# gargatik/Seamless-Through-Breaking-Rethinking-Image-Stitching-for-Optimal-Alignment

Hardware: AMD Instinct MI355X
Metric: stitched image-pairs/s at 512x512 (higher is better)
Workload: dtype f32 (decoder contractions, PatchEmbed's third conv and the C = 128 block tails: exact 3xbf16 split of both operands, 6 products on the bf16 matrix cores, fp32 accumulate -- error vs fp64 0.83x the fp32 MFMA chain's; everything else fp32); 1 GPU; UDIS-D-shaped 512x512 pairs, batch=1, FlowHomoAdpater.forward(type=test_eval); launch=hipGraph replay, pairs_in_flight=3

## Files before the change

include/stitch_gfx950.h:

```cpp
#ifndef STITCH_GFX950_H
#define STITCH_GFX950_H
#include <stdint.h>
#ifdef __cplusplus
extern "C" {
#endif

typedef struct st_gemm_desc {
    const float* a;
    const float* w;
    float* c;
    const float* bias;
    const float* aux0;
    const float* aux1;
    const float* aux2;
    const float* scale_ptr;
    int32_t M, N, K;
    int32_t H, W, Cin, ldx;
    int32_t kh, kw, sh, sw, ph, pw, Ho, Wo;
    int32_t ldw, ldc, ld_aux0, ld_aux1, ld_aux2;
    int32_t aux0_row_div, aux0_row_mod;
    int32_t act;
    int32_t epi;
    float alpha;
    int32_t batch;
// ... 92 lines not shown
int st_corr_volume_both_plan(int32_t B, int32_t N, int32_t C, int32_t aligned16);

int st_layernorm(const float* x, int32_t ldx, const float* w, const float* b, float* out, int32_t ldo,
                 int32_t rows, int32_t C, float eps, void* stream);
int st_softmax_rows(float* x, int32_t ld, int32_t rows, int32_t C, void* stream);
int st_l2norm_rows(const float* x, float* out, int32_t rows, int32_t C, void* stream);
int st_maxpool_nhwc(const float* x, float* out, int32_t B, int32_t H, int32_t W, int32_t C, int32_t k,
                    int32_t s, int32_t p, void* stream);
int st_dwconv3x3_residual(const float* x, const float* w, const float* bias, float* out, int32_t B,
                          int32_t H, int32_t W, int32_t C, void* stream);
int st_sine_pe(float* out, int32_t ld, int32_t rows, int32_t dim, const float* coords, int32_t ldc,
               int32_t Wg, int32_t ws, int32_t period, float cscale, float coff, int32_t accumulate,
               void* stream);
int st_attention_small(const float* q, int64_t q_bs, int64_t q_ts, const float* k, int64_t k_bs, int64_t k_ts,
                       const float* v, int64_t v_bs, int64_t v_ts, float* out, int64_t o_bs, int64_t o_ts,
                       int32_t B, int32_t heads, int32_t Nq, int32_t Nk, int32_t D, float scale, void* stream);
int st_attention_kvlds(const float* q, int64_t q_bs, int64_t q_ts, const float* k, int64_t k_bs, int64_t k_ts,
                       const float* v, int64_t v_bs, int64_t v_ts, float* out, int64_t o_bs, int64_t o_ts,
                       int32_t B, int32_t heads, int32_t Nq, int32_t Nk, int32_t D, float scale, void* stream);
int st_window_attention(const float* q, const float* k, const float* v, int64_t bs, int64_t ts,
                        const float* qpad, const float* kpad, const float* vpad, float* out, int64_t o_bs,
                        int64_t o_ts, int32_t B, int32_t H, int32_t W, int32_t heads, int32_t D, int32_t ws,
                        float scale, void* stream);
int st_ccl_softargmax(const float* G, float* out, int32_t ldo, int32_t B, int32_t h, int32_t w, void* stream);
int st_patch_conv1(const float* maps, const float* w36x16, const float* bias, float* out, int32_t M, int32_t H,
                   int32_t W, int32_t Ho, int32_t Wo, void* stream);
int st_patch_conv12(const float* cost_maps, const float* c0_w36x16, const float* c0_b, const float* c2_w32x576,
                    const float* c2_b, float* s2, int32_t M, int32_t H, int32_t W, void* stream);
int st_patch_conv12_planes(const float* cost_maps, const float* c0_w36x16, const float* c0_b, const float* c2_w32x576, const float* c2_b,
                           void* s2_planes, int64_t s2_pstride, int32_t M, int32_t H, int32_t W, void* stream);
int st_copy2d(const float* src, int32_t lds, float* dst, int32_t ldd, int32_t rows, int32_t cols, void* stream);
int st_prep_image(const float* src, float* dst, int32_t B, int32_t C, int32_t H, int32_t W, int32_t ldo,
                  float mul, float div, float sub, void* stream);

int st_latent_pool(const float* scores, int32_t ld_s, const float* tokens, int32_t ld_t, float* z, int32_t pixels,
                   int32_t P, void* stream);

int st_coords_grid(float* out, int32_t B, int32_t H, int32_t W, void* stream);
int st_coords_grid_init(float* out, const float* init, int32_t B, int32_t H, int32_t W, void* stream);
int st_flow_forward_interpolate(const float* src, int32_t src_is_coords_rows, float* out, int32_t B, int32_t H, int32_t W,
                                void* stream);
int st_flow_from_coords(const float* coords1, float* flow4, int32_t ld4, float* dst2, int32_t ld2, int32_t B,
                        int32_t H, int32_t W, void* stream);
int st_flow_encode(const float* coords1, const float* w98, const float* bias, float* out, int32_t ldo, float* flow2,
                   int32_t ld2, int32_t B, int32_t H, int32_t W, int32_t Co, void* stream);
int st_flow_encode_split3(const float* coords1, const float* w98, const float* bias, float* out, int32_t ldo, float* flow2,
                          int32_t ld2, int32_t B, int32_t H, int32_t W, int32_t Co, void* out_planes, int64_t out_pstride,
                          int64_t out_prows, void* flow_planes, int64_t flow_pstride, int64_t flow_prows, int32_t flow_col,
                          void* stream);
int st_cost_lookup(const float* maps, const float* coords, float* out, int32_t ldo, int32_t Nq, int32_t H2,
                   int32_t W2, int32_t r, void* stream);
int st_decoder_token_chain(float* corr, int32_t ld_corr, const float* coords1, const float* kv,
                           const float* const* weights16, int32_t rows, int32_t ntok, void* stream);
int st_convex_upsample(const float* coords1, const float* mask, int32_t ldm, float* out, int32_t B, int32_t H,
                       int32_t W, void* stream);

int st_dlt4(const float* src4x2, const float* motion, float* H, int32_t B, float mscale_x, float mscale_y,
            float div, void* stream);
int st_mat3_sandwich(const float* L, const float* X, const float* R, float* out, int32_t B, int32_t invert,
                     void* stream);
int st_homo_warp(const float* U, const float* theta, float* out, int32_t* idx, int32_t B, int32_t C,
                 int32_t n_ones, int32_t H, int32_t W, int32_t oh, int32_t ow, void* stream);
int st_mesh_bounds(const float* H, float* out4, int32_t B, float width, float height, int32_t gw, int32_t gh,
                   void* stream);
int st_flow_warp(const float* x, const float* flow, const float* mul, float* out, int32_t B, int32_t C,
                 int32_t H, int32_t W, void* stream);
int st_homo_flow_warp(const float* image2, const float* H8, const float* flow, float* out6, float* overlap, float* Hi,
                      int32_t B, int32_t H, int32_t W, void* stream);
int st_resize_bilinear(const float* x, float* out, int32_t planes, int32_t H, int32_t W, int32_t oh, int32_t ow,
                       int32_t align_corners, float div0, float div1, int32_t ndiv, void* stream);
int st_range_map(const float* flow, void* scratch_u64, float* out, int32_t B, int32_t H, int32_t W, void* stream);
int st_occlusion_from_range(const float* range, float* out, int64_t n, int32_t threshold, void* stream);
int st_morph_open(const float* mask, float* out, void* scratch_u8x2, int32_t N, int32_t H, int32_t W,
                  int32_t ksz, void* stream);
int st_eval_finish(float* final6, const float* occ, float* overlap, int32_t B, int32_t H, int32_t W, void* stream);
int st_blend(const float* homo1, const float* homo2, float* fin, const float* occ, float* output2, float* mask1,
             float* mask2, uint8_t* blend, int32_t h, int32_t w, void* stream);
int st_blend_plain(const float* homo1, const float* homo2, const float* fin, float* output2, float* mask1, float* mask2,
                   uint8_t* blend, int32_t h, int32_t w, void* stream);
int st_mean_threshold(const float* x, float* out, int32_t B, int32_t C, int32_t H, int32_t W, float thr,
                      void* stream);
int st_tps_solve_grid(const float* U, const float* source, const float* target, void* work_f64, float* T,
                      float* out, int32_t* idx, int32_t B, int32_t C, int32_t H, int32_t W, int32_t N,
                      int32_t oh, int32_t ow, void* stream);

int st_masked_psnr_ssim(const float* image1, const float* warped, int64_t warped_batch_stride, const float* maskmean,
                        void* partial_f64, double* out_psnr_ssim, int32_t B, int32_t H, int32_t W, void* stream);
int st_channel_mean(const float* x, int64_t batch_stride, float* out, int32_t B, int32_t C, int32_t H, int32_t W,
                    void* stream);

int st_load_rgb8(const void* src_u8_hwc, float* dst_chw, int32_t B, int32_t H, int32_t W, void* stream);

int st_jpeg_workspace_bytes(int32_t H, int32_t W, int32_t channels);
int st_jpeg_max_bytes(int32_t H, int32_t W, int32_t channels);
int st_jpeg_encode_u8(const void* src, int32_t H, int32_t W, int32_t channels, int64_t row_stride, void* out, int64_t out_capacity,
                      int32_t* out_nbytes, void* workspace, int64_t workspace_bytes, void* stream);

typedef struct st_jpeg_enc_params {
    int32_t quality;
    int32_t hs, vs;
    int32_t optimize;
    int32_t reserved[4];
} st_jpeg_enc_params;
int st_abi_jpeg_enc_params_size(void);
int st_jpeg_workspace_bytes_ex(int32_t H, int32_t W, int32_t channels, const st_jpeg_enc_params* params);
int st_jpeg_max_bytes_ex(int32_t H, int32_t W, int32_t channels, const st_jpeg_enc_params* params);
// ... 123 lines not shown
```

seamless-through-breaking-rethinking-image-stitching-for-optimal-alignment_amd/csrc/flowops.hip:

```cpp
#include "common.h"
#include <type_traits>
#include "../../include/stitch_gfx950.h"

__global__ void coords_grid_kernel(float* __restrict__ out, int B, int H, int W) {
    const size_t idx = (size_t)blockIdx.x * blockDim.x + threadIdx.x;
    if (idx >= (size_t)B * H * W) return;
    const int r = idx % ((size_t)H * W);
    out[idx * 2] = (float)(r % W);
    out[idx * 2 + 1] = (float)(r / W);
}

extern "C" int st_coords_grid(float* out, int32_t B, int32_t H, int32_t W, void* stream) {
    if (!out || B <= 0 || H <= 0 || W <= 0) return ST_EINVAL;
    const size_t total = (size_t)B * H * W;
    hipLaunchKernelGGL(coords_grid_kernel, dim3((total + 255) / 256), dim3(256), 0, (hipStream_t)stream, out, B, H, W);
    ST_CHECK_LAUNCH();
    return ST_OK;
}

__global__ void coords_grid_init_kernel(float* __restrict__ out, const float* __restrict__ init, int B, int H, int W) {
    const size_t idx = (size_t)blockIdx.x * blockDim.x + threadIdx.x;
    if (idx >= (size_t)B * H * W) return;
    const size_t N = (size_t)H * W, b = idx / N;
    const int r = idx % N;
// ... 109 lines not shown
                const unsigned nh = (unsigned)__builtin_amdgcn_update_dpp(0, (int)ph, 0xB1, 0xF, 0xF, false);
                const unsigned nm = (unsigned)__builtin_amdgcn_update_dpp(0, (int)pm, 0xB1, 0xF, 0xF, false);
                const unsigned nl = (unsigned)__builtin_amdgcn_update_dpp(0, (int)pl, 0xB1, 0xF, 0xF, false);
                if (!(c & 1)) {
                    unsigned* pp = reinterpret_cast<unsigned*>(out_planes + ((size_t)(c >> 5) * out_prows + img + (size_t)y * W + x) * 32 + (c & 31));
                    pp[0] = ph | (nh << 16); pp[out_pstride / 2] = pm | (nm << 16); pp[out_pstride] = pl | (nl << 16);
                }
            }
        }
    }
    if (flow2 && blockIdx.y == 0 && (wave & 1) == 0 && lane < 8 && tx * 8 + lane < W) {
        const float2 f = patch[(row + 3) * 14 + lane + 3];
        const size_t r = img + (size_t)y * W + tx * 8 + lane;
        flow2[r * ld2] = f.x; flow2[r * ld2 + 1] = f.y;
        if (flow_planes) {
            __bf16 hx, mx, lx, hy, my, ly;
            unsigned* pp = reinterpret_cast<unsigned*>(flow_planes + ((size_t)(flow_col >> 5) * flow_prows + r) * 32 + (flow_col & 31));
            st_split3(f.x, hx, mx, lx);
            st_split3(f.y, hy, my, ly);
            pp[0] = st_bf16_bits(hx) | ((unsigned)st_bf16_bits(hy) << 16);
            pp[flow_pstride / 2] = st_bf16_bits(mx) | ((unsigned)st_bf16_bits(my) << 16);
            pp[flow_pstride] = st_bf16_bits(lx) | ((unsigned)st_bf16_bits(ly) << 16);
        }
    }
}

extern "C" int st_flow_encode(const float* coords1, const float* w98, const float* bias, float* out, int32_t ldo, float* flow2,
                              int32_t ld2, int32_t B, int32_t H, int32_t W, int32_t Co, void* stream) {
    if (!coords1 || !w98 || !bias || !out || B <= 0 || H <= 0 || W <= 0 || Co <= 0 || (Co & 3) || ((uintptr_t)w98 & 15)) return ST_EINVAL;
    if (ldo < Co || (flow2 && ld2 < 2) || ((uintptr_t)coords1 & 7)) return ST_EINVAL;
    dim3 grid(((H + 3) / 4) * ((W + 7) / 8), (Co + 127) / 128, B);
    hipLaunchKernelGGL(flow_encode_kernel, grid, dim3(512), 0, (hipStream_t)stream, coords1, w98, bias, out, ldo, flow2, ld2, H, W, Co,
                       (__bf16*)nullptr, 0LL, 0LL, (__bf16*)nullptr, 0LL, 0LL, 0);
    ST_CHECK_LAUNCH();
    return ST_OK;
}

extern "C" int st_flow_encode_split3(const float* coords1, const float* w98, const float* bias, float* out, int32_t ldo, float* flow2,
                                     int32_t ld2, int32_t B, int32_t H, int32_t W, int32_t Co, void* out_planes, int64_t out_pstride,
                                     int64_t out_prows, void* flow_planes, int64_t flow_pstride, int64_t flow_prows, int32_t flow_col,
                                     void* stream) {
    if (!coords1 || !w98 || !bias || !out || B <= 0 || H <= 0 || W <= 0 || Co <= 0 || (Co & 31) || ((uintptr_t)w98 & 15)) return ST_EINVAL;
    if (ldo < Co || (flow2 && ld2 < 2) || ((uintptr_t)coords1 & 7)) return ST_EINVAL;
    if (!out_planes || out_pstride <= 0 || out_prows < (int64_t)B * H * W) return ST_EINVAL;
    if (flow_planes && (!flow2 || flow_pstride <= 0 || flow_prows < (int64_t)B * H * W || flow_col < 0 || (flow_col & 1))) return ST_EINVAL;
    dim3 grid(((H + 3) / 4) * ((W + 7) / 8), (Co + 127) / 128, B);
    hipLaunchKernelGGL(flow_encode_kernel, grid, dim3(512), 0, (hipStream_t)stream, coords1, w98, bias, out, ldo, flow2, ld2, H, W, Co,
                       (__bf16*)out_planes, (long long)out_pstride, (long long)out_prows, (__bf16*)flow_planes, (long long)flow_pstride,
                       (long long)flow_prows, (int)flow_col);
    ST_CHECK_LAUNCH();
    return ST_OK;
}

__global__ __launch_bounds__(256) void cost_lookup_kernel(const float* __restrict__ maps, const float* __restrict__ coords,
                                                          float* __restrict__ out, int ldo, int Nq, int H2, int W2, int r) {
#pragma clang fp contract(off)
    const int side = 2 * r + 1, nch = side * side;
    const size_t idx = (size_t)blockIdx.x * 256 + threadIdx.x;
    if (idx >= (size_t)Nq * nch) return;
    const int ch = idx % nch;
    const size_t n = idx / nch;
    const int i = ch / side, j = ch % side;
    const float x = coords[n * 2] + (float)(i - r);
    const float y = coords[n * 2 + 1] + (float)(j - r);
    const float gx = 2.0f * x / (float)(W2 - 1) - 1.0f, gy = 2.0f * y / (float)(H2 - 1) - 1.0f;
    const float ix = ((gx + 1.0f) / 2.0f) * (float)(W2 - 1), iy = ((gy + 1.0f) / 2.0f) * (float)(H2 - 1);
    const float x0f = floorf(ix), y0f = floorf(iy);
    const int x0 = (int)x0f, y0 = (int)y0f, x1 = x0 + 1, y1 = y0 + 1;
    const float x1f = x0f + 1.0f, y1f = y0f + 1.0f;
    const float nw = (x1f - ix) * (y1f - iy), ne = (ix - x0f) * (y1f - iy);
    const float sw = (x1f - ix) * (iy - y0f), se = (ix - x0f) * (iy - y0f);
    const float* m = maps + n * (size_t)(H2 * W2);
    const bool xin0 = x0 >= 0 && x0 < W2, xin1 = x1 >= 0 && x1 < W2;
    const bool yin0 = y0 >= 0 && y0 < H2, yin1 = y1 >= 0 && y1 < H2;
    float v = (xin0 && yin0 ? m[y0 * W2 + x0] : 0.f) * nw;
    v = __fmaf_rn(xin1 && yin0 ? m[y0 * W2 + x1] : 0.f, ne, v);
    v = __fmaf_rn(xin0 && yin1 ? m[y1 * W2 + x0] : 0.f, sw, v);
    v = __fmaf_rn(xin1 && yin1 ? m[y1 * W2 + x1] : 0.f, se, v);
    out[n * ldo + ch] = v;
}

extern "C" int st_cost_lookup(const float* maps, const float* coords, float* out, int32_t ldo, int32_t Nq, int32_t H2,
                              int32_t W2, int32_t r, void* stream) {
    if (!maps || !coords || !out || Nq <= 0 || r < 0 || r > 64 || ldo < (2 * r + 1) * (2 * r + 1)) return ST_EINVAL;
    if (H2 < 2 || W2 < 2 || (int64_t)H2 * W2 > 0x7fffffff) return ST_EINVAL;
    const size_t total = (size_t)Nq * (2 * r + 1) * (2 * r + 1);
    hipLaunchKernelGGL(cost_lookup_kernel, dim3((total + 255) / 256), dim3(256), 0, (hipStream_t)stream, maps, coords, out,
                       ldo, Nq, H2, W2, r);
    ST_CHECK_LAUNCH();
    return ST_OK;
}

__global__ __launch_bounds__(256) void convex_upsample_kernel(const float* __restrict__ coords1, const float* __restrict__ mask,
                                                              int ldm, float* __restrict__ out, int B, int H, int W) {
    const size_t gid = (size_t)blockIdx.x * 256 + threadIdx.x;
    const size_t pix = gid >> 6;
    if (pix >= (size_t)B * H * W) return;
    const int sub = gid & 63, i = sub >> 3, j = sub & 7;
    const int b = pix / ((size_t)H * W), r = pix % ((size_t)H * W);
    const int y = r / W, x = r % W;
    const float* mp = mask + pix * ldm + sub;
    float mv[9], mx = -INFINITY;
#pragma unroll
    for (int k = 0; k < 9; ++k) { mv[k] = mp[k * 64]; mx = fmaxf(mx, mv[k]); }
    float sum = 0.f;
#pragma unroll
    for (int k = 0; k < 9; ++k) { mv[k] = expf(mv[k] - mx); sum += mv[k]; }
    float ox = 0.f, oy = 0.f;
#pragma unroll
    for (int k = 0; k < 9; ++k) {
        const int yy = y + k / 3 - 1, xx = x + k % 3 - 1;
        const bool ok = yy >= 0 && yy < H && xx >= 0 && xx < W;
        const size_t p2 = ((size_t)b * H + min(max(yy, 0), H - 1)) * W + min(max(xx, 0), W - 1);
        const float2 cxy = *reinterpret_cast<const float2*>(coords1 + p2 * 2);
        const float okf = ok ? 8.0f : 0.0f;
        const float fx = okf * (cxy.x - (float)xx), fy = okf * (cxy.y - (float)yy);
        const float wgt = mv[k] / sum;
        ox += wgt * fx; oy += wgt * fy;
    }
    const size_t HW8 = (size_t)64 * H * W;
    const size_t o = (size_t)b * 2 * HW8 + (size_t)(8 * y + i) * (8 * W) + (8 * x + j);
    out[o] = ox;
    out[o + HW8] = oy;
}

extern "C" int st_convex_upsample(const float* coords1, const float* mask, int32_t ldm, float* out, int32_t B, int32_t H,
                                  int32_t W, void* stream) {
    if (!coords1 || !mask || !out || ldm < 576 || B <= 0 || H <= 0 || W <= 0 || ((uintptr_t)coords1 & 7)) return ST_EINVAL;
    const size_t total = (size_t)B * H * W * 64;
    hipLaunchKernelGGL(convex_upsample_kernel, dim3((total + 255) / 256), dim3(256), 0, (hipStream_t)stream, coords1, mask,
                       ldm, out, B, H, W);
    ST_CHECK_LAUNCH();
// ... 22 lines not shown
#pragma unroll
    for (int j = 0; j < K / 16; ++j) {
        const float4 a = *reinterpret_cast<const float4*>(X + i * LDX + 16 * j + 4 * g);
        float4 b[2];
#pragma unroll
        for (int t = 0; t < 2; ++t) b[t] = *reinterpret_cast<const float4*>(Wh + (16 * t + i) * LDWT + 16 * j + 4 * g);
#pragma unroll
        for (int t = 0; t < 2; ++t) acc[t] = __builtin_amdgcn_mfma_f32_16x16x4f32(a.x, b[t].x, acc[t], 0, 0, 0);
#pragma unroll
        for (int t = 0; t < 2; ++t) acc[t] = __builtin_amdgcn_mfma_f32_16x16x4f32(a.y, b[t].y, acc[t], 0, 0, 0);
#pragma unroll
        for (int t = 0; t < 2; ++t) acc[t] = __builtin_amdgcn_mfma_f32_16x16x4f32(a.z, b[t].z, acc[t], 0, 0, 0);
#pragma unroll
        for (int t = 0; t < 2; ++t) acc[t] = __builtin_amdgcn_mfma_f32_16x16x4f32(a.w, b[t].w, acc[t], 0, 0, 0);
    }
}

__device__ __forceinline__ void tc_store2(float* __restrict__ X, const f32x4 v[2], int col0, int lane) {
    const int c = lane & 15, g = lane >> 4;
#pragma unroll
    for (int t = 0; t < 2; ++t)
#pragma unroll
        for (int r = 0; r < 4; ++r) X[(4 * g + r) * TC_LDW + col0 + 16 * t + c] = v[t][r];
}

__device__ __forceinline__ void tc_layernorm2(f32x4 v[2], const float* __restrict__ w, const float* __restrict__ b, float* __restrict__ red_mine,
                                              const float* __restrict__ red_other, int col0, int lane) {
    const int c = lane & 15, g = lane >> 4;
    float mh[4], m2h[4];
#pragma unroll
    for (int r = 0; r < 4; ++r) {
        mh[r] = sum16(v[0][r] + v[1][r]) * (1.0f / 32.0f);
        const float d0 = v[0][r] - mh[r], d1 = v[1][r] - mh[r];
        m2h[r] = sum16(d0 * d0 + d1 * d1);
        if (c == 0) { red_mine[(4 * g + r) * 2] = mh[r]; red_mine[(4 * g + r) * 2 + 1] = m2h[r]; }
    }
    __syncthreads();
#pragma unroll
    for (int r = 0; r < 4; ++r) {
        const float mo = red_other[(4 * g + r) * 2], m2o = red_other[(4 * g + r) * 2 + 1];
        const float mean = 0.5f * (mh[r] + mo), d = mh[r] - mo;
        const float var = ((m2h[r] + m2o) + d * d * 16.0f) * (1.0f / 64.0f);
        const float rstd = 1.0f / sqrtf(var + 1e-5f);
#pragma unroll
        for (int t = 0; t < 2; ++t) v[t][r] = (v[t][r] - mean) * rstd * w[col0 + 16 * t + c] + b[col0 + 16 * t + c];
    }
}

template <int I, int N, class F>
__device__ __forceinline__ void tc_static_for(F&& f) {
    if constexpr (I < N) { f(std::integral_constant<int, I>{}); tc_static_for<I + 1, N>(f); }
}

template <int RG>
__global__ __launch_bounds__(128 * RG) void decoder_token_chain_kernel(float* __restrict__ corr, int ldc, const float* __restrict__ coords1,
                                                                       const float* __restrict__ kv, TokenChainArgs A, int rows, int ntok) {
    extern __shared__ __attribute__((aligned(16))) float sm[];
    float* W0 = sm;
    float* W2 = W0 + 64 * TC_LDW0;
    float* Wq = W2 + 64 * TC_LDW;
    float* Wp = Wq + 64 * TC_LDW;
    float* Wf0 = Wp + 64 * TC_LDW;
    float* Wf3 = Wf0 + 64 * TC_LDW;
    float* Vec = Wf3 + 64 * TC_LDW;
    float* Slab = Vec + 10 * 64;
    float* Red = Slab + RG * 16 * (TC_LDW0 + TC_LDW);
    const int tid = threadIdx.x, lane = tid & 63, wave = tid >> 6;
    constexpr int NT = 128 * RG;
    const int rg = wave >> 1, hf = wave & 1, col0 = 32 * hf;
    float* S0 = Slab + rg * 16 * (TC_LDW0 + TC_LDW);
    float* S1 = S0 + 16 * TC_LDW0;
    float* red_mine = Red + (rg * 2 + hf) * 32;
    const float* red_other = Red + (rg * 2 + (hf ^ 1)) * 32;
    const int row0 = (blockIdx.x * RG + rg) * 16;
    const int c = lane & 15, g = lane >> 4;
    const int jmax = ntok - 1;

    constexpr int P0 = 1536 / NT, P1 = 1024 / NT;
    float4 xv[3], w0v[P0];
    f32x4 wv[5 * P1], vecv;
    float cx[4], cy[4];
    {
        const int e = min(tid, 159), q = e >> 4;
        const float* vp = q == 0 ? A.b0 : q == 1 ? A.b2 : q == 2 ? A.n1w : q == 3 ? A.n1b : q == 4 ? A.bq : q == 5 ? A.bp : q == 6 ? A.n2w
                          : q == 7 ? A.n2b : q == 8 ? A.bf0 : A.bf3;
        vecv = *reinterpret_cast<const f32x4*>(vp + 4 * (e & 15));
    }
    tc_static_for<0, 3>([&](auto ic) {
        constexpr int i = decltype(ic)::value;
        const int e = (hf * 64 + lane) + 128 * i, r = e / 24, k4 = e % 24;
        xv[i] = *reinterpret_cast<const float4*>(corr + (size_t)min(row0 + r, rows - 1) * ldc + 4 * min(k4, 20));
    });
    tc_static_for<0, P0>([&](auto ic) {
        constexpr int i = decltype(ic)::value;
        const int e = tid + NT * i, n = e / 24, k4 = e % 24;
        w0v[i] = *reinterpret_cast<const float4*>(A.w0 + n * 84 + 4 * min(k4, 20));
    });
    tc_static_for<0, P1>([&](auto ic) {
        constexpr int i = decltype(ic)::value;
        const int off = 4 * (tid + NT * i);
        wv[5 * i + 0] = *reinterpret_cast<const f32x4*>(A.w2 + off);
        wv[5 * i + 1] = *reinterpret_cast<const f32x4*>(A.wq + off);
        wv[5 * i + 2] = *reinterpret_cast<const f32x4*>(A.wp + off);
        wv[5 * i + 3] = *reinterpret_cast<const f32x4*>(A.wf0 + off);
        wv[5 * i + 4] = *reinterpret_cast<const f32x4*>(A.wf3 + off);
    });
#pragma unroll
    for (int r = 0; r < 4; ++r) {
        const float2 p2 = *reinterpret_cast<const float2*>(coords1 + (size_t)min(row0 + 4 * g + r, rows - 1) * 2);
        cx[r] = p2.x; cy[r] = p2.y;
    }
    tc_static_for<0, 3>([&](auto ic) {
        constexpr int i = decltype(ic)::value;
        const int e = (hf * 64 + lane) + 128 * i, r = e / 24, k4 = e % 24;
        *reinterpret_cast<float4*>(S0 + r * TC_LDW0 + 4 * k4) = k4 < 21 ? xv[i] : make_float4(0.f, 0.f, 0.f, 0.f);
    });
    tc_static_for<0, P0>([&](auto ic) {
        constexpr int i = decltype(ic)::value;
        const int e = tid + NT * i, n = e / 24, k4 = e % 24;
        *reinterpret_cast<float4*>(W0 + n * TC_LDW0 + 4 * k4) = k4 < 21 ? w0v[i] : make_float4(0.f, 0.f, 0.f, 0.f);
    });
    tc_static_for<0, P1>([&](auto ic) {
        constexpr int i = decltype(ic)::value;
        const int e = tid + NT * i, n = e >> 4, k4 = e & 15, off = n * TC_LDW + 4 * k4;
        *reinterpret_cast<f32x4*>(W2 + off) = wv[5 * i + 0];
        *reinterpret_cast<f32x4*>(Wq + off) = wv[5 * i + 1];
        *reinterpret_cast<f32x4*>(Wp + off) = wv[5 * i + 2];
        *reinterpret_cast<f32x4*>(Wf0 + off) = wv[5 * i + 3];
        *reinterpret_cast<f32x4*>(Wf3 + off) = wv[5 * i + 4];
    });
    if (tid < 160) *reinterpret_cast<f32x4*>(Vec + 4 * tid) = vecv;
    asm volatile("" ::: "memory");
    const int head = 4 * hf + g;
    float4 kk[8][2], vv[8][2];
    {
        const float* kvr = kv + (size_t)min(row0 + c, rows - 1) * ntok * 128 + 8 * head;
#pragma unroll
        for (int j = 0; j < 8; ++j)
#pragma unroll
            for (int e = 0; e < 2; ++e) kk[j][e] = *reinterpret_cast<const float4*>(kvr + min(j, jmax) * 128 + 4 * e);
#pragma unroll
        for (int j = 0; j < 8; ++j)
#pragma unroll
            for (int e = 0; e < 2; ++e) vv[j][e] = *reinterpret_cast<const float4*>(kvr + min(j, jmax) * 128 + 64 + 4 * e);
    }
    asm volatile("" ::: "memory");
    __syncthreads();
    const float *b0 = Vec, *b2 = Vec + 64, *n1w = Vec + 128, *n1b = Vec + 192, *bq = Vec + 256, *bp = Vec + 320, *n2w = Vec + 384,
                *n2b = Vec + 448, *bf0 = Vec + 512, *bf3 = Vec + 576;
    f32x4 acc[2], query[2], x[2];
    tc_gemm2<96, TC_LDW0, TC_LDW0>(S0, W0 + col0 * TC_LDW0, acc, lane);
#pragma unroll
    for (int t = 0; t < 2; ++t)
#pragma unroll
        for (int r = 0; r < 4; ++r) acc[t][r] = st_act(acc[t][r] + b0[col0 + 16 * t + c], ST_ACT_GELU);
    tc_store2(S1, acc, col0, lane);
    __syncthreads();
    tc_gemm2<64, TC_LDW, TC_LDW>(S1, W2 + col0 * TC_LDW, query, lane);
#pragma unroll
    for (int t = 0; t < 2; ++t)
#pragma unroll
        for (int r = 0; r < 4; ++r) query[t][r] += b2[col0 + 16 * t + c];
#pragma unroll
    for (int t = 0; t < 2; ++t) acc[t] = query[t];
    tc_layernorm2(acc, n1w, n1b, red_mine, red_other, col0, lane);
// ... 25 lines not shown
            float a0 = 0.f;
            const float kf[8] = {kk[j][0].x, kk[j][0].y, kk[j][0].z, kk[j][0].w, kk[j][1].x, kk[j][1].y, kk[j][1].z, kk[j][1].w};
#pragma unroll
            for (int e = 0; e < 8; ++e) a0 = fmaf(qv[e], kf[e], a0);
            s0[j] = j < ntok ? a0 * scale : -INFINITY;
        }
        float m0 = s0[0];
#pragma unroll
        for (int j = 1; j < 8; ++j) m0 = fmaxf(m0, s0[j]);
        float d0 = 0.f;
#pragma unroll
        for (int e = 0; e < 8; ++e) o[e] = 0.f;
#pragma unroll
        for (int j = 0; j < 8; ++j) {
            const float p0 = expf(s0[j] - m0);
            d0 += p0;
            const float vf[8] = {vv[j][0].x, vv[j][0].y, vv[j][0].z, vv[j][0].w, vv[j][1].x, vv[j][1].y, vv[j][1].z, vv[j][1].w};
#pragma unroll
            for (int e = 0; e < 8; ++e) o[e] = fmaf(p0, vf[e], o[e]);
        }
        const float i0 = 1.0f / d0;
        __builtin_amdgcn_wave_barrier();
        *reinterpret_cast<float4*>(S1 + c * TC_LDW + 8 * head) = make_float4(o[0] * i0, o[1] * i0, o[2] * i0, o[3] * i0);
        *reinterpret_cast<float4*>(S1 + c * TC_LDW + 8 * head + 4) = make_float4(o[4] * i0, o[5] * i0, o[6] * i0, o[7] * i0);
    }
    __syncthreads();
    tc_gemm2<64, TC_LDW, TC_LDW>(S1, Wp + col0 * TC_LDW, acc, lane);
#pragma unroll
    for (int t = 0; t < 2; ++t)
#pragma unroll
        for (int r = 0; r < 4; ++r) x[t][r] = query[t][r] + (acc[t][r] + bp[col0 + 16 * t + c]);
#pragma unroll
    for (int t = 0; t < 2; ++t) acc[t] = x[t];
    tc_layernorm2(acc, n2w, n2b, red_mine, red_other, col0, lane);
    tc_store2(S0, acc, col0, lane);
    __syncthreads();
    tc_gemm2<64, TC_LDW, TC_LDW>(S0, Wf0 + col0 * TC_LDW, acc, lane);
#pragma unroll
    for (int t = 0; t < 2; ++t)
#pragma unroll
        for (int r = 0; r < 4; ++r) acc[t][r] = st_act(acc[t][r] + bf0[col0 + 16 * t + c], ST_ACT_GELU);
    tc_store2(S1, acc, col0, lane);
    __syncthreads();
    tc_gemm2<64, TC_LDW, TC_LDW>(S1, Wf3 + col0 * TC_LDW, acc, lane);
#pragma unroll
    for (int t = 0; t < 2; ++t)
#pragma unroll
        for (int r = 0; r < 4; ++r) {
            const int row = row0 + 4 * g + r;
            if (row < rows) corr[(size_t)row * ldc + 84 + col0 + 16 * t + c] = x[t][r] + (acc[t][r] + bf3[col0 + 16 * t + c]);
        }
}

extern "C" int st_decoder_token_chain(float* corr, int32_t ld_corr, const float* coords1, const float* kv, const float* const* weights16,
                                      int32_t rows, int32_t ntok, void* stream) {
    if (!corr || !coords1 || !kv || !weights16 || rows <= 0 || ntok <= 0 || ntok > 8 || ld_corr < 148 || (ld_corr & 3)) return ST_EINVAL;
    TokenChainArgs A;
    const float** dst = reinterpret_cast<const float**>(&A);
    for (int i = 0; i < 16; ++i) { if (!weights16[i]) return ST_EINVAL; dst[i] = weights16[i]; }
    constexpr int RG = 4;
    const size_t lds = (size_t)(64 * TC_LDW0 + 5 * 64 * TC_LDW + 640 + RG * 16 * (TC_LDW0 + TC_LDW) + RG * 64) * sizeof(float);
    (void)hipFuncSetAttribute((const void*)decoder_token_chain_kernel<RG>, hipFuncAttributeMaxDynamicSharedMemorySize, (int)lds);
    hipLaunchKernelGGL(decoder_token_chain_kernel<RG>, dim3((rows + 16 * RG - 1) / (16 * RG)), dim3(128 * RG), lds, (hipStream_t)stream, corr, ld_corr,
                       coords1, kv, A, rows, ntok);
    ST_CHECK_LAUNCH();
    return ST_OK;
}
```

seamless-through-breaking-rethinking-image-stitching-for-optimal-alignment_amd/flowformer.py:

```python
from __future__ import annotations

import os

import torch
import torch.nn as nn

from . import ops
from .checkpoint import HP, ParamTree, flat_params, flow_spec
from .homography import pack_conv


SPLIT3 = os.environ.get("ST_SPLIT3", "1") != "0"


def _new(rows, cols, dev, zero=False):
    return (torch.zeros if zero else torch.empty)((rows, cols), device=dev, dtype=torch.float32)


def _planes_copy(p):
    return ops.Planes(p.rows, p.C, None, t=p.t.clone(), c0=p.c0, ncols=p.ncols)


def _keep(trace, **named):
    if trace is None:
# ... 490 lines not shown
        gru = (S["zbuf"], gru_tab["1"], gru_tab["2"], *((D["s3"] if s3 else D)[k] for k in ("zr1", "q1", "zr2", "q2")), B, H1, W1)
        if s3:
            ops.sepconv_gru_split3(hxA, S["hxA_p"], S["hxB_p"], *gru)
        else:
            ops.sepconv_gru(hxA, S["hxB"], *gru)
        _keep(trace, gru=net)
        ops.conv_gemm(_act(S, "hxA", 0, 128), _wt(D, S, "fh1"), S["fh"], geom=g3, bias=D["fh1"][1], act="relu")
        ops.conv_gemm(S["fh"], D["fh2"][0], coords1, geom=g3, bias=D["fh2"][1], epi="add", aux1=coords1)
        _keep(trace, fh=S["fh"], coords_out=coords1, hxA=hxA)
        if s3:
            _keep(trace, planes={k: S[k] for k in ("hxA_p", "cor1_p", "flo1_p", "corflo_p")})

    def _mask_head(self, S, B, H1, W1, trace=None):
        D = self._pk["dec"]
        ops.conv_gemm(_act(S, "hxA", 0, 128), _wt(D, S, "m0"), S["fh"], geom=(B, H1, W1, 3, 3, 1, 1, 1, 1), bias=D["m0"][1], act="relu")
        _keep(trace, mask_hidden=S["fh"])
        mask = _new(S["hxA"].shape[0], 576, S["hxA"].device)
        ops.conv_gemm(S["fh"], D["m2"][0], mask, bias=D["m2"][1], alpha=0.25)
        return mask

    def _decoder_prologue(self, ctx, B, H1, W1, trace=None):
        D = self._pk["dec"]
        dev = ctx.device
        N = H1 * W1
        R = B * N
        S = self._update_state(R, B, N, dev)
        inp = _new(R, 128, dev)
        ops.conv_gemm(ctx, D["proj_net"][0], S["hxA"][:, :128], bias=D["proj_net"][1], act="tanh", **_emit(S, "hxA", 0, 128))
        ops.conv_gemm(ctx, D["proj_inp"][0], inp, bias=D["proj_inp"][1], act="relu")
        gru_tab = self._gru_tables(inp, B, H1, W1)
        qk = _new(R, 256, dev)
        attn = torch.empty((B, N, N), device=dev)
        ops.gma_attention(inp, D["qk"], qk, attn, B, N)
        _keep(trace, net=S["hxA"][:, :128], inp=inp, gru_tab=gru_tab, attn=attn, qk=qk)
        if S["s3"]:
            _keep(trace, net_p=S["hxA_p"])
        return dict(S=S, inp=inp, gru_tab=gru_tab, attn=attn, qk=qk)

    def _decoder(self, mem, ctx, cost_maps, B, H1, W1, iters, trace=None, flow_init=None):
        D = self._pk["dec"]
        dev = ctx.device
        N = H1 * W1
        R = B * N
        nl = self._pk["latents"].shape[0]
        pro = None if trace is None else trace[-1].setdefault("prologue", {})
        pre = self._decoder_prologue(ctx, B, H1, W1, trace=pro)
        S, gru_tab, attn = pre["S"], pre["gru_tab"], pre["attn"]
        kv = _new(R * nl, 128, dev)
        ops.conv_gemm(mem, D["ca"]["kv"][0], kv, bias=D["ca"]["kv"][1])
        _keep(pro, kv=kv)
        coords1 = _new(R, 2, dev)
        ops.coords_grid(coords1, B, H1, W1, init=flow_init)
        for it in range(iters):
            ops.cost_lookup9x9(cost_maps, coords1, S["corr"], R, H1, W1)
            ops.decoder_token_chain(S["corr"], coords1, kv, D["chain16"], R, nl)
            rec = _record(trace)
            self._update_block(S, coords1, attn, gru_tab, B, H1, W1, trace=rec)
            _keep(rec, coords1=coords1, net=S["hxA"][:, :128], corr=S["corr"])
        last = None if trace is None else trace[-1]
        mask = self._mask_head(S, B, H1, W1, trace=last)
        flow_up = torch.empty((B, 2, 8 * H1, 8 * W1), device=dev)
        ops.convex_upsample(coords1, mask, flow_up, B, H1, W1)
        _keep(last, mask=mask, flow_up=flow_up)
        return flow_up, coords1

    def _forward(self, image1, image2, iters, trace, flow_init, pair):
        if not image1.is_cuda:
            raise RuntimeError("FlowFormer runs on the MI355X HIP kernels only: move the module and inputs to cuda")
        pk = self._pk or self.pack()
        iters = HP["decoder_depth"] if iters is None else iters
        B, _, H, W = image1.shape
        if H % 32 or W % 32:
            raise RuntimeError(f"input size {H}x{W} must be a multiple of 32 (reference runs both nets at 512x512)")
        dev = image1.device
        Bd = 2 * B if pair else B
        tr = None if trace is None else dict(cnet=[], fnet=[], encoder={})
        x = _new(2 * B * H * W, 4, dev)
        ops.prep_image(image1.contiguous(), x[:B * H * W], 4, 2.0, 255.0, 1.0)
        ops.prep_image(image2.contiguous(), x[B * H * W:], 4, 2.0, 255.0, 1.0)
        ctx, H1, W1 = self._twins(pk["cnet"], x if pair else x[:B * H * W], Bd, H, W, trace=tr and tr["cnet"])
        feats, _, _ = self._twins(pk["fnet"], x, 2 * B, H, W, trace=tr and tr["fnet"])
        N = H1 * W1
        feats = feats.view(2, B, N, 256)
        cost_maps = torch.empty((Bd * N, N), device=dev)
        if pair:
            ops.corr_volume_both(feats[0], feats[1], cost_maps[:B * N].view(B, N, N), cost_maps[B * N:].view(B, N, N))
        else:
            ops.corr_volume(feats[0], feats[1], cost_maps.view(B, N, N))
        mem = self._cost_encoder(cost_maps, ctx, Bd, H1, W1, trace=tr and tr["encoder"])
        if trace is not None:
            trace.append(dict(context=ctx, feats=feats, cost_maps=cost_maps, mem=mem, **tr))
        flow_up, coords1 = self._decoder(mem, ctx, cost_maps, Bd, H1, W1, iters, trace, flow_init=flow_init)
        return flow_up, coords1, (Bd, H1, W1)

    def flow_rows(self, image1, image2, iters=None, trace=None, flow_init=None):
        return self._forward(image1, image2, iters, trace, flow_init, pair=False)

    def flow_rows_pair(self, image_a, image_b, iters=None, trace=None, flow_init=None):
        return self._forward(image_a, image_b, iters, trace, flow_init, pair=True)

    def forward(self, image1, image2, mask=None, output=None, flow_init=None):
        if flow_init is not None:
            flow_init = flow_init.to(image1.device, torch.float32).contiguous()
        flow_up, coords1, (B, H1, W1) = self.flow_rows(image1, image2, flow_init=flow_init)
        flow4 = _new(B * H1 * W1, 4, flow_up.device)
        ops.flow_from_coords(coords1, flow4, None, B, H1, W1)
        low = flow4[:, :2].reshape(B, H1, W1, 2).permute(0, 3, 1, 2).contiguous()
        return flow_up, low
# ... 9 lines not shown
```

seamless-through-breaking-rethinking-image-stitching-for-optimal-alignment_amd/ops.py:

```python
from __future__ import annotations

import ctypes as C

import torch

from ._lib import ChainDesc, GemmDesc, JpegDecParams, JpegEncParams, MlpDesc, check, lib
from .jpeg_probe import JpegInfo, probe as _jpeg_probe
from ._lib import StitchError as StitchErrorBase

ACT = dict(none=0, relu=1, gelu=2, sigmoid=3, tanh=4, lrelu=5)
EPI = dict(store=0, add=1, mul=2, gru=3, axpy=4, zr=5)

assert lib.st_abi_gemm_desc_size() == C.sizeof(GemmDesc), "st_gemm_desc ABI mismatch between header and binding"
assert lib.st_abi_chain_desc_size() == C.sizeof(ChainDesc), "st_chain_desc ABI mismatch between header and binding"
assert lib.st_abi_mlp_desc_size() == C.sizeof(MlpDesc), "st_mlp_desc ABI mismatch between header and binding"
assert lib.st_abi_jpeg_dec_params_size() == C.sizeof(JpegDecParams), "st_jpeg_dec_params ABI mismatch between header and binding"
assert lib.st_abi_jpeg_enc_params_size() == C.sizeof(JpegEncParams), "st_jpeg_enc_params ABI mismatch between header and binding"


def _stream():
    return C.c_void_p(torch.cuda.current_stream().cuda_stream)


def _p(t):
# ... 369 lines not shown
    if tuple(init.shape) != (B, 2, H, W) or init.dtype != torch.float32 or not init.is_contiguous() or init.device != out.device:
        raise ValueError(f"flow_init must be a contiguous float32 [{B}, 2, {H}, {W}] tensor on {out.device}")
    check(lib.st_coords_grid_init(_p(out), _p(init), B, H, W, _stream()), "st_coords_grid_init")


def forward_interpolate(flow, out=None, *, coords_rows=None):
    if coords_rows is None:
        B, two, H, W = flow.shape
        ok = two == 2
    else:
        B, H, W = coords_rows
        ok = tuple(flow.shape) == (B * H * W, 2)
    if not ok or flow.dtype != torch.float32 or not flow.is_contiguous() or not flow.is_cuda:
        raise ValueError("forward_interpolate takes a contiguous float32 cuda tensor [B,2,H1,W1], or coords1 rows [B*H1*W1,2]")
    if out is None:
        out = torch.empty((B, 2, H, W), device=flow.device)
    elif tuple(out.shape) != (B, 2, H, W) or out.dtype != torch.float32 or not out.is_contiguous() or out.device != flow.device:
        raise ValueError(f"out must be a contiguous float32 [{B}, 2, {H}, {W}] tensor on {flow.device}")
    check(lib.st_flow_forward_interpolate(_p(flow), 0 if coords_rows is None else 1, _p(out), B, H, W, _stream()),
          "st_flow_forward_interpolate")
    return out


def flow_from_coords(coords1, flow4, dst2, B, H, W):
    check(lib.st_flow_from_coords(_p(coords1), _p(flow4), _ld(flow4) if flow4 is not None else 0, _p(dst2),
                                  _ld(dst2) if dst2 is not None else 0, B, H, W, _stream()), "st_flow_from_coords")


def flow_encode(coords1, w98, bias, out, flow2, B, H, W):
    check(lib.st_flow_encode(_pc(coords1), _pc(w98), _pc(bias), _p(out), _ld(out), _p(flow2), _ld(flow2) if flow2 is not None else 0,
                             B, H, W, w98.shape[1], _stream()), "st_flow_encode")
    return out


def flow_encode_split3(coords1, w98, bias, out, flow2, B, H, W, out_planes, flow_planes):
    fp, fcol = flow_planes
    check(lib.st_flow_encode_split3(_pc(coords1), _pc(w98), _pc(bias), _p(out), _ld(out), _p(flow2), _ld(flow2), B, H, W, w98.shape[1],
                                    C.c_void_p(out_planes.ptr()), out_planes.pstride, out_planes.rows,
                                    C.c_void_p(fp.t.data_ptr()), fp.pstride, fp.rows, int(fcol), _stream()), "st_flow_encode_split3")
    return out


def cost_lookup(maps, coords, out, Nq, H2, W2, r=4):
    check(lib.st_cost_lookup(_p(maps), _p(coords), _p(out), _ld(out), Nq, H2, W2, r, _stream()), "st_cost_lookup")
    return out


def decoder_token_chain(corr, coords1, kv, weights16, rows, ntok):
    arr = (C.c_void_p * 16)(*[w.data_ptr() for w in weights16])
    check(lib.st_decoder_token_chain(_p(corr), _ld(corr), _pc(coords1), _p(kv), arr, rows, ntok, _stream()), "st_decoder_token_chain")
    return corr


def _ws(dev):
    ws = _workspace(dev)
    return ws.data_ptr(), ws.numel()


def patch_conv12(maps, c0_w, c0_b, c2_w, c2_b, out, M, H=64, W=64):
    check(lib.st_patch_conv12(_pc(maps), _pc(c0_w), _pc(c0_b), _pc(c2_w), _pc(c2_b), _p(out), M, H, W, _stream()), "st_patch_conv12")
    return out


def cost_lookup9x9(maps, coords, out, Nq, H2, W2):
    check(lib.st_cost_lookup9x9(_p(maps), _pc(coords), _p(out), _ld(out), Nq, H2, W2, _stream()), "st_cost_lookup9x9")
    return out


def patch_embed(cost_maps, weights11, ld_f0, pe_bias, s1, s2, s3, s4, tokens, M, H, W):
    arr = (C.c_void_p * 11)(*[w.data_ptr() for w in weights11])

    def call(s1_):
        return lib.st_patch_embed(_pc(cost_maps), arr, ld_f0, _pc(pe_bias), _pc(s1_) if s1_ is not None else None, _pc(s2), _pc(s3), _pc(s4), _pc(tokens),
                                  M, H, W, *_ws(cost_maps.device), _stream())
    rc = call(s1)
    if rc == 1001 and s1 is None:
        Hp, Wp = (H + 7) // 8 * 8, (W + 7) // 8 * 8
        rc = call(torch.empty((M * (Hp // 2) * (Wp // 2), 16), device=cost_maps.device, dtype=torch.float32))
    check(rc, "st_patch_embed")
    return tokens


def pe_tail_split3_pack(w_f0, w_f2):
    assert w_f0.shape[0] == 128 and w_f0.shape[1] >= 64 and w_f0.stride(1) == 1 and w_f2.shape == (128, 128) and w_f2.is_contiguous()
    nb = C.c_int64(0)
    check(lib.st_pe_tail_split3_image_bytes(C.byref(nb)), "st_pe_tail_split3_image_bytes")
    img = torch.empty(nb.value, dtype=torch.uint8, device=w_f0.device)
    check(lib.st_pe_tail_split3_pack(_p(w_f0), w_f0.stride(0), _p(w_f2), C.c_void_p(img.data_ptr()), nb.value, _stream()), "st_pe_tail_split3_pack")
    return img


def pe_tail_split3(x, tab, image, b2, gamma, beta, out, eps=1e-5):
    assert x.shape[1] == 64 and x.is_contiguous() and out.shape == (x.shape[0], 128) and out.is_contiguous() and tab.shape[1] == 128 and tab.is_contiguous()
    check(lib.st_pe_tail_split3(_p(x), _p(tab), tab.shape[0], C.c_void_p(image.data_ptr()), image.numel(), _p(b2), _p(gamma), _p(beta), float(eps), _p(out),
                                x.shape[0], _stream()), "st_pe_tail_split3")
    return out


def patch_embed_split3(cost_maps, weights11, ld_f0, pe_bias, s2_planes, c4_w_planes, s3, s4, tokens, M, H, W, tail_image=None):
    arr = (C.c_void_p * 11)(*[w.data_ptr() for w in weights11])
    check(lib.st_patch_embed_split3(_pc(cost_maps), arr, ld_f0, _pc(pe_bias), C.c_void_p(s2_planes.ptr()), s2_planes.pstride, C.c_void_p(c4_w_planes.ptr()),
                                    c4_w_planes.pstride, _pc(s3), _pc(s4) if s4 is not None else None, _pc(tokens), M, H, W,
                                    C.c_void_p(tail_image.data_ptr()) if tail_image is not None else None, tail_image.numel() if tail_image is not None else 0,
                                    *_ws(cost_maps.device), _stream()), "st_patch_embed_split3")
    return tokens

# ... 690 lines not shown
```

Baseline: 94.48 pairs/s.

## Fuse 9x9 cost-volume lookup into decoder token-chain kernel

The per-iteration bilinear 9x9 cost lookup is folded into the decoder token-chain kernel. Each workgroup computes per-axis offsets and weights into LDS, gathers the four map samples per tap, blends them, and writes them straight into the LDS slab while still storing corr to global memory. This removes one kernel launch per decoder iteration and the global round trip of the corr tile. In exchange the kernel uses more registers and LDS, and the scattered map gathers now sit inside the chain kernel's prologue.

New measurement: 94.94 pairs/s, median of 6. About the same (+0.5%).

```diff
diff --git a/include/stitch_gfx950.h b/include/stitch_gfx950.h
--- a/include/stitch_gfx950.h
+++ b/include/stitch_gfx950.h
@@ -168,6 +168,8 @@
                    int32_t W2, int32_t r, void* stream);
 int st_decoder_token_chain(float* corr, int32_t ld_corr, const float* coords1, const float* kv,
                            const float* const* weights16, int32_t rows, int32_t ntok, void* stream);
+int st_decoder_lookup_chain(const float* cost_maps, float* corr, int32_t ld_corr, const float* coords1, const float* kv,
+                            const float* const* weights16, int32_t rows, int32_t H2, int32_t W2, int32_t ntok, void* stream);
 int st_convex_upsample(const float* coords1, const float* mask, int32_t ldm, float* out, int32_t B, int32_t H,
                        int32_t W, void* stream);
 
diff --git a/seamless-through-breaking-rethinking-image-stitching-for-optimal-alignment_amd/csrc/flowops.hip b/seamless-through-breaking-rethinking-image-stitching-for-optimal-alignment_amd/csrc/flowops.hip
--- a/seamless-through-breaking-rethinking-image-stitching-for-optimal-alignment_amd/csrc/flowops.hip
+++ b/seamless-through-breaking-rethinking-image-stitching-for-optimal-alignment_amd/csrc/flowops.hip
@@ -185,32 +185,47 @@
     return ST_OK;
 }
 
+struct CostAxis {
+    int i0;
+    float w0, w1;
+};
+
+__device__ __forceinline__ CostAxis cost_lookup_axis(float c, int d, int r, int n) {
+#pragma clang fp contract(off)
+    const float a = c + (float)(d - r);
+    const float g = 2.0f * a / (float)(n - 1) - 1.0f;
+    const float p = ((g + 1.0f) / 2.0f) * (float)(n - 1);
+    const float f0 = floorf(p), f1 = f0 + 1.0f;
+    CostAxis t;
+    t.i0 = (int)f0; t.w0 = f1 - p; t.w1 = p - f0;
+    return t;
+}
+
+__device__ __forceinline__ float cost_lookup_blend(const CostAxis& x, const CostAxis& y, float m_nw, float m_ne, float m_sw, float m_se) {
+#pragma clang fp contract(off)
+    const float nw = x.w0 * y.w0, ne = x.w1 * y.w0, sw = x.w0 * y.w1, se = x.w1 * y.w1;
+    float v = m_nw * nw;
+    v = __fmaf_rn(m_ne, ne, v);
+    v = __fmaf_rn(m_sw, sw, v);
+    v = __fmaf_rn(m_se, se, v);
+    return v;
+}
+
 __global__ __launch_bounds__(256) void cost_lookup_kernel(const float* __restrict__ maps, const float* __restrict__ coords,
                                                           float* __restrict__ out, int ldo, int Nq, int H2, int W2, int r) {
-#pragma clang fp contract(off)
     const int side = 2 * r + 1, nch = side * side;
     const size_t idx = (size_t)blockIdx.x * 256 + threadIdx.x;
     if (idx >= (size_t)Nq * nch) return;
     const int ch = idx % nch;
     const size_t n = idx / nch;
     const int i = ch / side, j = ch % side;
-    const float x = coords[n * 2] + (float)(i - r);
-    const float y = coords[n * 2 + 1] + (float)(j - r);
-    const float gx = 2.0f * x / (float)(W2 - 1) - 1.0f, gy = 2.0f * y / (float)(H2 - 1) - 1.0f;
-    const float ix = ((gx + 1.0f) / 2.0f) * (float)(W2 - 1), iy = ((gy + 1.0f) / 2.0f) * (float)(H2 - 1);
-    const float x0f = floorf(ix), y0f = floorf(iy);
-    const int x0 = (int)x0f, y0 = (int)y0f, x1 = x0 + 1, y1 = y0 + 1;
-    const float x1f = x0f + 1.0f, y1f = y0f + 1.0f;
-    const float nw = (x1f - ix) * (y1f - iy), ne = (ix - x0f) * (y1f - iy);
-    const float sw = (x1f - ix) * (iy - y0f), se = (ix - x0f) * (iy - y0f);
+    const CostAxis ax = cost_lookup_axis(coords[n * 2], i, r, W2), ay = cost_lookup_axis(coords[n * 2 + 1], j, r, H2);
+    const int x0 = ax.i0, y0 = ay.i0, x1 = x0 + 1, y1 = y0 + 1;
     const float* m = maps + n * (size_t)(H2 * W2);
     const bool xin0 = x0 >= 0 && x0 < W2, xin1 = x1 >= 0 && x1 < W2;
     const bool yin0 = y0 >= 0 && y0 < H2, yin1 = y1 >= 0 && y1 < H2;
-    float v = (xin0 && yin0 ? m[y0 * W2 + x0] : 0.f) * nw;
-    v = __fmaf_rn(xin1 && yin0 ? m[y0 * W2 + x1] : 0.f, ne, v);
-    v = __fmaf_rn(xin0 && yin1 ? m[y1 * W2 + x0] : 0.f, sw, v);
-    v = __fmaf_rn(xin1 && yin1 ? m[y1 * W2 + x1] : 0.f, se, v);
-    out[n * ldo + ch] = v;
+    out[n * ldo + ch] = cost_lookup_blend(ax, ay, xin0 && yin0 ? m[y0 * W2 + x0] : 0.f, xin1 && yin0 ? m[y0 * W2 + x1] : 0.f,
+                                          xin0 && yin1 ? m[y1 * W2 + x0] : 0.f, xin1 && yin1 ? m[y1 * W2 + x1] : 0.f);
 }
 
 extern "C" int st_cost_lookup(const float* maps, const float* coords, float* out, int32_t ldo, int32_t Nq, int32_t H2,
@@ -339,9 +354,10 @@
     if constexpr (I < N) { f(std::integral_constant<int, I>{}); tc_static_for<I + 1, N>(f); }
 }
 
-template <int RG>
+template <int RG, bool LOOKUP>
 __global__ __launch_bounds__(128 * RG) void decoder_token_chain_kernel(float* __restrict__ corr, int ldc, const float* __restrict__ coords1,
-                                                                       const float* __restrict__ kv, TokenChainArgs A, int rows, int ntok) {
+                                                                       const float* __restrict__ kv, TokenChainArgs A, int rows, int ntok,
+                                                                       const float* __restrict__ maps, int mapH, int mapW) {
     extern __shared__ __attribute__((aligned(16))) float sm[];
     float* W0 = sm;
     float* W2 = W0 + 64 * TC_LDW0;
@@ -351,11 +367,12 @@
     float* Wf3 = Wf0 + 64 * TC_LDW;
     float* Vec = Wf3 + 64 * TC_LDW;
     float* Slab = Vec + 10 * 64;
-    float* Red = Slab + RG * 16 * (TC_LDW0 + TC_LDW);
+    constexpr int SLAB = 16 * (TC_LDW0 + TC_LDW) + (LOOKUP ? 64 : 0);
+    float* Red = Slab + RG * SLAB;
     const int tid = threadIdx.x, lane = tid & 63, wave = tid >> 6;
     constexpr int NT = 128 * RG;
     const int rg = wave >> 1, hf = wave & 1, col0 = 32 * hf;
-    float* S0 = Slab + rg * 16 * (TC_LDW0 + TC_LDW);
+    float* S0 = Slab + rg * SLAB;
     float* S1 = S0 + 16 * TC_LDW0;
     float* red_mine = Red + (rg * 2 + hf) * 32;
     const float* red_other = Red + (rg * 2 + (hf ^ 1)) * 32;
@@ -367,13 +384,49 @@
     float4 xv[3], w0v[P0];
     f32x4 wv[5 * P1], vecv;
     float cx[4], cy[4];
+    constexpr int NS = 11, NA = 3;
+    const int l128 = hf * 64 + lane;
+    float axc[NA];
+    float padv;
+    if constexpr (LOOKUP) {
+#pragma unroll
+        for (int k = 0; k < NA; ++k) {
+            const int e = min(l128 + 128 * k, 287), a = e / 144, r = (e - 144 * a) / 9;
+            axc[k] = coords1[(size_t)min(row0 + r, rows - 1) * 2 + a];
+        }
+        const int e = min(l128, 47);
+        padv = corr[(size_t)min(row0 + e / 3, rows - 1) * ldc + 81 + e % 3];
+    }
+    uint4* Ax = reinterpret_cast<uint4*>(S1);
+    float mv[NS][4];
+    if constexpr (LOOKUP) {
+#pragma unroll
+        for (int k = 0; k < NA; ++k) {
+            const int e = l128 + 128 * k, ec = min(e, 287), a = ec / 144, d = (ec - 144 * a) % 9;
+            const int n = a ? mapH : mapW, st = a ? mapW : 1;
+            const CostAxis t = cost_lookup_axis(axc[k], d, 4, n);
+            const int i0 = t.i0, i1 = i0 + 1;
+            const unsigned oa = (unsigned)(min(max(i0, 0), n - 1) * st) | (i0 >= 0 && i0 < n ? 0x80000000u : 0u);
+            const unsigned ob = (unsigned)(min(max(i1, 0), n - 1) * st) | (i1 >= 0 && i1 < n ? 0x80000000u : 0u);
+            if (e < 288) Ax[e] = make_uint4(oa, ob, __float_as_uint(t.w0), __float_as_uint(t.w1));
+        }
+        __syncthreads();
+#pragma unroll
+        for (int k = 0; k < NS; ++k) {
+            const int s = min(l128 + 128 * k, 1295), r = s / 81, ch = s - 81 * r, i = ch / 9, j = ch - 9 * i;
+            const uint2 ox = *reinterpret_cast<const uint2*>(Ax + 9 * r + i), oy = *reinterpret_cast<const uint2*>(Ax + 144 + 9 * r + j);
+            const float* m = maps + (size_t)min(row0 + r, rows - 1) * (size_t)(mapH * mapW);
+            const unsigned xa = ox.x & 0x7fffffffu, xb = ox.y & 0x7fffffffu, ya = oy.x & 0x7fffffffu, yb = oy.y & 0x7fffffffu;
+            mv[k][0] = m[ya + xa]; mv[k][1] = m[ya + xb]; mv[k][2] = m[yb + xa]; mv[k][3] = m[yb + xb];
+        }
+    }
     {
         const int e = min(tid, 159), q = e >> 4;
         const float* vp = q == 0 ? A.b0 : q == 1 ? A.b2 : q == 2 ? A.n1w : q == 3 ? A.n1b : q == 4 ? A.bq : q == 5 ? A.bp : q == 6 ? A.n2w
                           : q == 7 ? A.n2b : q == 8 ? A.bf0 : A.bf3;
         vecv = *reinterpret_cast<const f32x4*>(vp + 4 * (e & 15));
     }
-    tc_static_for<0, 3>([&](auto ic) {
+    if constexpr (!LOOKUP) tc_static_for<0, 3>([&](auto ic) {
         constexpr int i = decltype(ic)::value;
         const int e = (hf * 64 + lane) + 128 * i, r = e / 24, k4 = e % 24;
         xv[i] = *reinterpret_cast<const float4*>(corr + (size_t)min(row0 + r, rows - 1) * ldc + 4 * min(k4, 20));
@@ -397,7 +450,31 @@
         const float2 p2 = *reinterpret_cast<const float2*>(coords1 + (size_t)min(row0 + 4 * g + r, rows - 1) * 2);
         cx[r] = p2.x; cy[r] = p2.y;
     }
-    tc_static_for<0, 3>([&](auto ic) {
+    if constexpr (LOOKUP) {
+        asm volatile("" ::: "memory");
+#pragma unroll
+        for (int k = 0; k < NS; ++k) {
+            const int s = min(l128 + 128 * k, 1295), r = s / 81, ch = s - 81 * r, i = ch / 9, j = ch - 9 * i;
+            const uint4 ex = Ax[9 * r + i], ey = Ax[144 + 9 * r + j];
+            CostAxis ax, ay;
+            ax.i0 = 0; ay.i0 = 0;
+            ax.w0 = __uint_as_float(ex.z); ax.w1 = __uint_as_float(ex.w); ay.w0 = __uint_as_float(ey.z); ay.w1 = __uint_as_float(ey.w);
+            const unsigned mxa = (unsigned)((int)ex.x >> 31), mxb = (unsigned)((int)ex.y >> 31);
+            const unsigned mya = (unsigned)((int)ey.x >> 31), myb = (unsigned)((int)ey.y >> 31);
+            const float v = cost_lookup_blend(ax, ay, __uint_as_float(__float_as_uint(mv[k][0]) & mxa & mya), __uint_as_float(__float_as_uint(mv[k][1]) & mxb & mya),
+                                              __uint_as_float(__float_as_uint(mv[k][2]) & mxa & myb), __uint_as_float(__float_as_uint(mv[k][3]) & mxb & myb));
+            if (l128 + 128 * k < 1296) {
+                S0[r * TC_LDW0 + ch] = v;
+                if (row0 + r < rows) corr[(size_t)(row0 + r) * ldc + ch] = v;
+            }
+        }
+        if (l128 < 48) {
+            float* p = S0 + (l128 / 3) * TC_LDW0;
+            p[81 + l128 % 3] = padv;
+            *reinterpret_cast<float4*>(p + 84 + 4 * (l128 % 3)) = make_float4(0.f, 0.f, 0.f, 0.f);
+        }
+    }
+    if constexpr (!LOOKUP) tc_static_for<0, 3>([&](auto ic) {
         constexpr int i = decltype(ic)::value;
         const int e = (hf * 64 + lane) + 128 * i, r = e / 24, k4 = e % 24;
         *reinterpret_cast<float4*>(S0 + r * TC_LDW0 + 4 * k4) = k4 < 21 ? xv[i] : make_float4(0.f, 0.f, 0.f, 0.f);
@@ -529,17 +606,29 @@
         }
 }
 
-extern "C" int st_decoder_token_chain(float* corr, int32_t ld_corr, const float* coords1, const float* kv, const float* const* weights16,
-                                      int32_t rows, int32_t ntok, void* stream) {
+template <bool LOOKUP>
+static int launch_token_chain(const float* maps, float* corr, int32_t ld_corr, const float* coords1, const float* kv,
+                              const float* const* weights16, int32_t rows, int32_t H2, int32_t W2, int32_t ntok, void* stream) {
     if (!corr || !coords1 || !kv || !weights16 || rows <= 0 || ntok <= 0 || ntok > 8 || ld_corr < 148 || (ld_corr & 3)) return ST_EINVAL;
+    if (LOOKUP && (!maps || H2 < 2 || W2 < 2 || (int64_t)H2 * W2 > 0x7fffffff)) return ST_EINVAL;
     TokenChainArgs A;
     const float** dst = reinterpret_cast<const float**>(&A);
     for (int i = 0; i < 16; ++i) { if (!weights16[i]) return ST_EINVAL; dst[i] = weights16[i]; }
     constexpr int RG = 4;
-    const size_t lds = (size_t)(64 * TC_LDW0 + 5 * 64 * TC_LDW + 640 + RG * 16 * (TC_LDW0 + TC_LDW) + RG * 64) * sizeof(float);
-    (void)hipFuncSetAttribute((const void*)decoder_token_chain_kernel<RG>, hipFuncAttributeMaxDynamicSharedMemorySize, (int)lds);
-    hipLaunchKernelGGL(decoder_token_chain_kernel<RG>, dim3((rows + 16 * RG - 1) / (16 * RG)), dim3(128 * RG), lds, (hipStream_t)stream, corr, ld_corr,
-                       coords1, kv, A, rows, ntok);
-    ST_CHECK_LAUNCH();
-    return ST_OK;
-}
+    const size_t lds = (size_t)(64 * TC_LDW0 + 5 * 64 * TC_LDW + 640 + RG * (16 * (TC_LDW0 + TC_LDW) + (LOOKUP ? 64 : 0)) + RG * 64) * sizeof(float);
+    (void)hipFuncSetAttribute((const void*)decoder_token_chain_kernel<RG, LOOKUP>, hipFuncAttributeMaxDynamicSharedMemorySize, (int)lds);
+    hipLaunchKernelGGL((decoder_token_chain_kernel<RG, LOOKUP>), dim3((rows + 16 * RG - 1) / (16 * RG)), dim3(128 * RG), lds, (hipStream_t)stream,
+                       corr, ld_corr, coords1, kv, A, rows, ntok, maps, H2, W2);
+    ST_CHECK_LAUNCH();
+    return ST_OK;
+}
+
+extern "C" int st_decoder_token_chain(float* corr, int32_t ld_corr, const float* coords1, const float* kv, const float* const* weights16,
+                                      int32_t rows, int32_t ntok, void* stream) {
+    return launch_token_chain<false>(nullptr, corr, ld_corr, coords1, kv, weights16, rows, 0, 0, ntok, stream);
+}
+
+extern "C" int st_decoder_lookup_chain(const float* cost_maps, float* corr, int32_t ld_corr, const float* coords1, const float* kv,
+                                       const float* const* weights16, int32_t rows, int32_t H2, int32_t W2, int32_t ntok, void* stream) {
+    return launch_token_chain<true>(cost_maps, corr, ld_corr, coords1, kv, weights16, rows, H2, W2, ntok, stream);
+}
diff --git a/seamless-through-breaking-rethinking-image-stitching-for-optimal-alignment_amd/flowformer.py b/seamless-through-breaking-rethinking-image-stitching-for-optimal-alignment_amd/flowformer.py
--- a/seamless-through-breaking-rethinking-image-stitching-for-optimal-alignment_amd/flowformer.py
+++ b/seamless-through-breaking-rethinking-image-stitching-for-optimal-alignment_amd/flowformer.py
@@ -566,8 +566,7 @@
         coords1 = _new(R, 2, dev)
         ops.coords_grid(coords1, B, H1, W1, init=flow_init)
         for it in range(iters):
-            ops.cost_lookup9x9(cost_maps, coords1, S["corr"], R, H1, W1)
-            ops.decoder_token_chain(S["corr"], coords1, kv, D["chain16"], R, nl)
+            ops.decoder_lookup_chain(cost_maps, S["corr"], coords1, kv, D["chain16"], R, H1, W1, nl)
             rec = _record(trace)
             self._update_block(S, coords1, attn, gru_tab, B, H1, W1, trace=rec)
             _keep(rec, coords1=coords1, net=S["hxA"][:, :128], corr=S["corr"])
diff --git a/seamless-through-breaking-rethinking-image-stitching-for-optimal-alignment_amd/ops.py b/seamless-through-breaking-rethinking-image-stitching-for-optimal-alignment_amd/ops.py
--- a/seamless-through-breaking-rethinking-image-stitching-for-optimal-alignment_amd/ops.py
+++ b/seamless-through-breaking-rethinking-image-stitching-for-optimal-alignment_amd/ops.py
@@ -445,6 +445,13 @@
     return corr
 
 
+def decoder_lookup_chain(cost_maps, corr, coords1, kv, weights16, rows, H2, W2, ntok):
+    arr = (C.c_void_p * 16)(*[w.data_ptr() for w in weights16])
+    check(lib.st_decoder_lookup_chain(_p(cost_maps), _p(corr), _ld(corr), _pc(coords1), _p(kv), arr, rows, H2, W2, ntok, _stream()),
+          "st_decoder_lookup_chain")
+    return corr
+
+
 def _ws(dev):
     ws = _workspace(dev)
     return ws.data_ptr(), ws.numel()
```
